# JeremyWesthead/deacon-server

Measured on AMD Instinct MI355X. Metric: Mbp/s filtered (k=31,w=15 vs panhuman-1-sized index), decisions bit-exact vs CPU, higher is better.
Workload: dtype u64

## Files before the change

deacon-server_amd/csrc/ctx.hip:

```cpp
#include "dcn_ctx.h"
#include "dcn_host_pool.h"

#include <atomic>
#include <cstdlib>
#include <cstring>
#include <mutex>
#include <new>

using dcn_host::HostPool;

uint32_t dcn_cu_count() {
    int dev = 0, cus = 256;
    if (hipGetDevice(&dev) == hipSuccess) (void)hipDeviceGetAttribute(&cus, hipDeviceAttributeMultiprocessorCount, dev);
    return (uint32_t)std::max(cus, 1);
}

namespace dcn_impl {

int alloc_records(dcn_ctx *c, uint64_t n_records) {
    n_records = (n_records + 63) / 64 * 64;
    if (n_records > (1ull << 29)) return dcn_fail(DCN_ERR_CAPACITY, "more than 2^29 hit records in global sets per batch: use smaller batches");
    if (c->d_set_slots) hipFree(c->d_set_slots);
    c->d_set_slots = nullptr;
    c->rec_capacity = 0;
    DCN_TRY(dev_alloc(&c->d_set_slots, 4 * n_records + 64, "set_slots"));
    c->rec_capacity = n_records;
    return DCN_OK;
}

void free_slot_buffers(dcn_slot &sl) {
    if (sl.owns_buffers) {
        void *dev[] = {sl.d_ascii, sl.d_packed, sl.d_invmask, sl.d_offsets, sl.d_unit_id, sl.d_keep, sl.d_hits, sl.d_total};
        for (void *p : dev)
            if (p) hipFree(p);
    }
    if (sl.d_report) hipFree(sl.d_report);
    if (sl.d_off32) hipFree(sl.d_off32);
    if (sl.d_mask_pairs) hipFree(sl.d_mask_pairs);
    void *host[] = {sl.h_keep, sl.h_hits, sl.h_total, sl.h_report, sl.h_off32, sl.h_mask_pairs};
    for (void *p : host)
        if (p) hipHostFree(p);
    if (sl.done) hipEventDestroy(sl.done);
    for (hipEvent_t e : sl.ev_h2d) hipEventDestroy(e);
    for (hipEvent_t e : sl.ev_comp) hipEventDestroy(e);
    sl = dcn_slot();
}

static void free_ctx(dcn_ctx *c) {
    if (!c) return;
    hipSetDevice(c->device);
    if (c->stream) hipStreamSynchronize(c->stream);
    if (c->copy_stream) hipStreamSynchronize(c->copy_stream);
    if (c->d2h_stream) hipStreamSynchronize(c->d2h_stream);
    if (c->pack_stream) {
        hipStreamSynchronize(c->pack_stream);
        hipStreamDestroy(c->pack_stream);
    }
    for (int i = 0; i < 2; ++i) {
        if (c->pack_done[i]) hipEventDestroy(c->pack_done[i]);
        if (c->buf_free[i]) hipEventDestroy(c->buf_free[i]);
    }
    if (c->plan_done) hipEventDestroy(c->plan_done);
    if (c->d_packed_b) hipFree(c->d_packed_b);
    if (c->d_invmask_b) hipFree(c->d_invmask_b);
    if (c->d_pack_status) hipFree(c->d_pack_status);
    for (auto &sl : c->slots) free_slot_buffers(sl);
    void *dev[] = {c->d_ascii, c->d_offsets, c->d_unit_id, c->d_packed, c->d_invmask,
                   c->d_read_tiles, c->d_read_tile_first, c->d_unit_first_read, c->d_unit_tile_first, c->d_unit_tile_count, c->d_tiles,
                   c->d_keep, c->d_unit_state, c->d_hits, c->d_total, c->d_unit_scratch, c->d_caps,
                   c->d_set_off, c->d_tile_hits, c->d_pending, c->d_big, c->d_rec_hash, c->d_set_slots, c->d_status, c->d_wave_kept, c->d_report, c->d_dump_hash,
                   c->d_dump_pos, c->d_dump_count, c->d_dump_valid, c->d_tile_read_pos,
                   c->d_cls_big, c->d_cls_n_big, c->d_cls_match, c->d_cls_hits, c->d_cls_total,
                   c->d_loc_bits, c->d_loc_labels, c->d_loc_counts, c->d_loc_big, c->d_loc_n_big, c->d_loc_block_sums,
                   c->d_loc_seg_offsets, c->d_loc_segs, c->d_trk_bin_offsets, c->d_trk_piece_offsets, c->d_trk_bins,
                   c->d_plc_words, c->d_plc_abits, c->d_plc_big, c->d_plc_n_big, c->d_plc_out,
                   c->d_pls_rbits, c->d_pls_n_rounds, c->d_pls_read_counts, c->d_pls_counts, c->d_pls_block_sums,
                   c->d_pls_offsets, c->d_pls_rounds, c->d_pls_out, c->d_ppr_out, c->d_ppr_hist, c->d_vfy_items, c->d_vfy_out,
                   c->d_aln_work, c->d_aln_n_ops, c->d_aln_trace, c->d_aln_slots, c->d_aln_cigar, c->d_aln_offsets, c->d_aln_block_sums};
    for (void *p : dev)
        if (p && !((char *)p >= c->d_slab && (char *)p < c->d_slab + c->slab_bytes)) hipFree(p);
    if (c->d_slab) hipFree(c->d_slab);
    for (int i = 0; i < dcn_ctx::N_STAGE; ++i) {
        if (c->h_stage[i]) hipHostFree(c->h_stage[i]);
        if (c->stage_free[i]) hipEventDestroy(c->stage_free[i]);
    }
    for (int i = 0; i < dcn_ctx::N_EV; ++i) {
        if (c->ev_h2d[i]) hipEventDestroy(c->ev_h2d[i]);
        if (c->ev_comp[i]) hipEventDestroy(c->ev_comp[i]);
    }
    if (c->h_report) hipHostFree(c->h_report);
    for (int i = 0; i < dcn_ctx::PROF_RING; ++i)
        for (int j = 0; j <= DCN_N_STAGES; ++j)
            if (c->prof_ev[i][j]) hipEventDestroy(c->prof_ev[i][j]);
    if (c->copy_done) hipEventDestroy(c->copy_done);
    if (c->stream) hipStreamDestroy(c->stream);
    if (c->copy_stream) hipStreamDestroy(c->copy_stream);
    if (c->d2h_stream) hipStreamDestroy(c->d2h_stream);
    delete c;
}

static int prof_harvest(dcn_ctx *c, int only_slot = -1) {
    for (int i = 0; i < dcn_ctx::PROF_RING; ++i) {
        if (!c->prof_used[i] || (only_slot >= 0 && i != only_slot)) continue;
        const int first = c->prof_scan_only[i] ? DCN_STAGE_SCAN : 0, last = c->prof_scan_only[i] ? DCN_STAGE_SCAN : DCN_N_STAGES - 1;
        DCN_HIP(hipEventSynchronize(c->prof_ev[i][last + 1]));
        for (int j = first; j <= last; ++j) {
            float ms = 0.f;
            DCN_HIP(hipEventElapsedTime(&ms, c->prof_ev[i][j], c->prof_ev[i][j + 1]));
            c->prof_ms[j] += ms;
        }
// ... 4 lines not shown
}

int prof_begin(dcn_ctx *c, int *slot) {
    *slot = -1;
    if (!c->profiling) return DCN_OK;
    int i = c->prof_next;
    c->prof_next = (i + 1) % dcn_ctx::PROF_RING;
    if (c->prof_used[i]) DCN_TRY(prof_harvest(c, i));
    for (int j = 0; j <= DCN_N_STAGES; ++j)
        if (!c->prof_ev[i][j]) DCN_HIP(hipEventCreate(&c->prof_ev[i][j]));
    c->prof_scan_only[i] = c->profiling == 2;
    if (c->profiling == 1) DCN_HIP(hipEventRecord(c->prof_ev[i][0], c->stream));
    *slot = i;
    return DCN_OK;
}

int check_params(const dcn_params *p) {
    if (!p) return dcn_fail(DCN_ERR_ARG, "params is NULL");
    if (p->reserved != 0) return dcn_fail(DCN_ERR_ARG, "params.reserved must be 0");
    if (p->deplete > 1) return dcn_fail(DCN_ERR_ARG, "params.deplete must be 0 or 1");
    return DCN_OK;
}

static bool ensure_pack_ahead(dcn_ctx *c) {
    if (c->pack_ahead_state != 0) return c->pack_ahead_state > 0;
    c->pack_ahead_state = -1;
    if (!getenv("DCN_PACK_AHEAD") || getenv("DCN_NO_PACK_AHEAD")) return false;
    int prio_low = 0, prio_high = 0;
    (void)hipDeviceGetStreamPriorityRange(&prio_low, &prio_high);
    bool ok = hipStreamCreateWithPriority(&c->pack_stream, hipStreamNonBlocking, prio_high) == hipSuccess;
    ok = ok && hipEventCreateWithFlags(&c->plan_done, hipEventDisableTiming) == hipSuccess;
    for (int i = 0; ok && i < 2; ++i)
        ok = hipEventCreateWithFlags(&c->pack_done[i], hipEventDisableTiming) == hipSuccess &&
             hipEventCreateWithFlags(&c->buf_free[i], hipEventDisableTiming) == hipSuccess;
    ok = ok && hipMalloc((void **)&c->d_packed_b, packed_words(c->max_bases) * sizeof(uint32_t)) == hipSuccess &&
         hipMalloc((void **)&c->d_invmask_b, mask_words(c->max_bases) * sizeof(uint32_t)) == hipSuccess &&
         hipMalloc((void **)&c->d_pack_status, 2 * sizeof(dcn_status)) == hipSuccess;
    if (ok) {
        ok = hipMemset(c->d_packed_b, 0, packed_words(c->max_bases) * sizeof(uint32_t)) == hipSuccess &&
             hipMemset(c->d_invmask_b, 0, mask_words(c->max_bases) * sizeof(uint32_t)) == hipSuccess &&
             hipDeviceSynchronize() == hipSuccess;
    }
    if (!ok) {
        (void)hipGetLastError();
        if (c->d_packed_b) hipFree(c->d_packed_b);
        if (c->d_invmask_b) hipFree(c->d_invmask_b);
        if (c->d_pack_status) hipFree(c->d_pack_status);
        c->d_packed_b = c->d_invmask_b = nullptr;
        c->d_pack_status = nullptr;
        return false;
    }
    c->pack_ahead_state = 1;
    return true;
}

static dcn_scan_args scan_args(const dcn_ctx *c, const dcn_index *index, uint32_t *packed, uint32_t *invmask, uint64_t stream_bases);

int enqueue_batch(dcn_ctx *c, const BatchView &v, const dcn_params *params, bool pack_ahead) {
    hipStream_t st = c->stream;
    const dcn_index *idx = c->index;
    if (c->scratch_dirty) DCN_HIP(hipMemsetAsync(c->d_unit_scratch, 0, (uint64_t)c->max_reads * 4 * sizeof(uint32_t), st));
    c->scratch_dirty = true;
    DCN_HIP(hipMemsetAsync(c->d_status, 0, sizeof(dcn_status), st));

    int prof_slot = -1;
    DCN_TRY(prof_begin(c, &prof_slot));
    uint32_t *packed = v.d_packed + DCN_FRONT_PAD, *invmask = v.d_invmask + DCN_FRONT_PAD;
    int ahead_buf = -1;
    const uint32_t *newline_flag = nullptr;
    bool short_fused = false;
    static const bool no_early_out = getenv("DCN_NO_EARLY_OUT") != nullptr, no_early_out_pairs = getenv("DCN_NO_EARLY_OUT_PAIRS") != nullptr;
    const bool decisions_only_call = !v.d_hits && !v.d_total && params->abs_threshold >= 1 && params->abs_threshold <= 4 && !no_early_out;
    if (v.d_ascii && pack_ahead && c->profiling != 1 && ensure_pack_ahead(c)) {
        ahead_buf = c->pack_buf;
        c->pack_buf ^= 1;
        if (ahead_buf == 1) {
            packed = c->d_packed_b + DCN_FRONT_PAD;
            invmask = c->d_invmask_b + DCN_FRONT_PAD;
        }
        dcn_status *ps = c->d_pack_status + ahead_buf;
        DCN_HIP(hipStreamWaitEvent(c->pack_stream, c->buf_free[ahead_buf], 0));
        if (!getenv("DCN_PACK_AHEAD_EARLY")) DCN_HIP(hipStreamWaitEvent(c->pack_stream, c->plan_done, 0));
        DCN_HIP(hipMemsetAsync(ps, 0, sizeof(dcn_status), c->pack_stream));
        DCN_TRY(dcn_launch_pack_beside(v.d_ascii, v.b0, v.b1, packed, invmask, ps, c->pack_stream));
        DCN_HIP(hipEventRecord(c->pack_done[ahead_buf], c->pack_stream));
        DCN_HIP(hipStreamWaitEvent(st, c->pack_done[ahead_buf], 0));
        newline_flag = &ps->any_newline;
    } else if (v.d_ascii) {
        short_fused = c->short_fused && !v.d_unit_id && params->prefix_length == 0 && v.b0 == 0 && v.b1 == v.stream_bases &&
                      v.n_reads == v.n_units && c->tile_windows >= dcn_short_lmax() && idx->variant == DCN_VARIANT_DEFAULT &&
                      dcn_scan_has_short_path(idx->k, idx->w) && !decisions_only_call;
        if (short_fused) DCN_TRY(dcn_launch_shape(v.d_offsets, v.n_reads, v.stream_bases, dcn_short_lmax(), c->d_status, st));
        DCN_TRY(dcn_launch_pack(v.d_ascii, v.b0, v.b1, packed, invmask, c->d_status, st));
    }
    DCN_PROF_MARK(DCN_STAGE_PACK);

    const uint32_t n_reads = v.n_reads, n_units = v.n_units;
    dcn_plan_args pa = plan_args(c, idx, v.d_ascii, v.d_offsets, v.d_unit_id, n_reads, n_units, params->prefix_length);
    pa.unit_base = v.unit_base;
    pa.unit_state = c->d_unit_state;
    pa.unit_scratch = c->d_unit_scratch;
    pa.scratch_stride = c->max_reads;
    pa.newline_flag = newline_flag;
    pa.stream_bases = v.stream_bases;
    pa.check_offsets = 1;
    pa.max_tiles = c->max_tiles;
    pa.short_armed = short_fused ? 1u : 0u;
    DCN_TRY(dcn_launch_plan(pa, st));
    if (pack_ahead && c->pack_ahead_state == 1) DCN_HIP(hipEventRecord(c->plan_done, st));
    DCN_PROF_MARK(DCN_STAGE_PLAN);

    const UnitScratch us = unit_scratch(c);
    dcn_scan_args sa = scan_args(c, idx, packed, invmask, v.stream_bases);
    sa.unit_tile_first = c->d_unit_tile_first;
    sa.unit_tile_count = c->d_unit_tile_count;
    sa.abs_threshold = params->abs_threshold;
    sa.rel_threshold = params->rel_threshold;
    sa.deplete = params->deplete;
    sa.early_out_max_items = 0;
    if (decisions_only_call) {
        uint32_t lo = 0, hi = 65535;
        while (lo < hi) {
            uint32_t mid = (lo + hi + 1) / 2;
            if (dcn_required_hits(params->abs_threshold, params->rel_threshold, mid) == params->abs_threshold) lo = mid;
            else hi = mid - 1;
        }
        sa.early_out_max_items = lo;
        sa.early_out_pairs = no_early_out_pairs ? 0u : 1u;
    }
    sa.keep = v.d_keep;
    sa.hits = v.d_hits;
    sa.total = v.d_total;
    sa.unit_state = c->d_unit_state;
    sa.g_total = us.g_total;
    sa.g_hitcnt = us.g_hitcnt;
    sa.g_zero = us.g_zero;
    sa.rec_hash = c->d_rec_hash;
    sa.rec_shift = c->rec_shift;
    sa.tile_windows = c->tile_windows;
    sa.tile_hits = c->d_tile_hits;
    sa.pending = c->d_pending;
    sa.status = c->d_status;
    sa.ascii = short_fused ? v.d_ascii : nullptr;
    sa.offsets = v.d_offsets;
    sa.n_reads = n_reads;
    sa.wave_kept = c->d_wave_kept;
    DCN_TRY(dcn_launch_scan(sa, tile_bound(c, n_reads, v.b1 - v.b0), false, st));
    DCN_PROF_MARK(DCN_STAGE_SCAN);

    const bool decisions_only = !v.d_hits && !v.d_total && !getenv("DCN_NO_EARLY_OUT");
    const dcn_distinct_args da = distinct_args(c, n_units, params, c->d_rec_hash, c->rec_shift, decisions_only ? us.g_total : nullptr);
    DCN_TRY(dcn_launch_distinct(da, st));
    DCN_PROF_MARK(DCN_STAGE_DISTINCT);

    dcn_finish_args fa = finish_args(c, n_units, params, v.d_unit_id ? c->d_unit_first_read : nullptr, v.d_offsets, v.d_keep,
                                     v.d_hits, v.d_total, v.d_report);
    fa.short_counted = short_fused ? 1u : 0u;
    fa.pending = c->d_pending;
    fa.wave_kept = c->d_wave_kept;
    DCN_TRY(dcn_launch_finish(fa, st));
    c->scratch_dirty = false;
    if (pack_ahead && c->pack_ahead_state == 1) DCN_HIP(hipEventRecord(c->buf_free[ahead_buf >= 0 ? ahead_buf : 0], st));
    DCN_PROF_MARK(DCN_STAGE_FINISH);
    if (prof_slot >= 0) c->prof_used[prof_slot] = true;
    return DCN_OK;
}

int grow_run_slots(dcn_ctx *c) {
    if (c->rec_shift == 0) return DCN_OK;
    const bool in_slab = c->d_rec_hash && (char *)c->d_rec_hash >= c->d_slab && (char *)c->d_rec_hash < c->d_slab + c->slab_bytes;
    if (c->d_rec_hash && !in_slab) hipFree(c->d_rec_hash);
    c->d_rec_hash = nullptr;
    const uint32_t old_shift = c->rec_shift;
    c->rec_shift = 0;
    int rc = dev_alloc(&c->d_rec_hash, c->max_bases + 128, "rec_hash (one slot per window)");
    if (rc != DCN_OK) {
        c->rec_shift = old_shift;
        int rc2 = dev_alloc(&c->d_rec_hash, (c->max_bases >> old_shift) + 256, "rec_hash");
        return rc2 != DCN_OK ? rc2 : rc;
    }
    static std::atomic<bool> said{false};
    if (!said.exchange(true) && getenv("DCN_QUIET") == nullptr)
        std::fprintf(stderr, "deacon-hip: a unit's hits outgrew its run of the record array; this context now keeps one slot per window "
                             "(%.2f GB instead of %.2f GB of device memory)\n", (c->max_bases + 128) * 8e-9,
                     ((c->max_bases >> old_shift) + 256) * 8e-9);
    return DCN_OK;
}

int overflow_error(const dcn_ctx *c, uint64_t need) {
    return dcn_fail(DCN_ERR_CAPACITY, "hit-record scratch overflow: need " + std::to_string(need) +
                                          " records, have " + std::to_string(c->rec_capacity) +
                                          " (dcn_ctx_reserve_records)");
}

int sync_and_check(dcn_ctx *c, uint64_t *needed_records) {
    DCN_HIP(hipStreamSynchronize(c->stream));
    if (needed_records) *needed_records = 0;
    if (c->profiling) DCN_TRY(prof_harvest(c));
    if (!c->batch_pending) return DCN_OK;
    c->batch_pending = false;
// ... 320 lines not shown
}

}

using namespace dcn_impl;

extern "C" int dcn_ctx_create(const dcn_index *index, uint64_t max_batch_bases, uint32_t max_batch_reads,
                              dcn_ctx **out) {
    if (!out) return dcn_fail(DCN_ERR_ARG, "out is NULL");
    *out = nullptr;
    if (!index) return dcn_fail(DCN_ERR_ARG, "index is NULL");
    if (max_batch_bases == 0 || max_batch_reads == 0) return dcn_fail(DCN_ERR_ARG, "batch limits must be > 0");
    if (max_batch_reads > 0xFFFFFF00u) return dcn_fail(DCN_ERR_ARG, "max_batch_reads too large");
    dcn_ctx *c = new (std::nothrow) dcn_ctx();
    if (!c) return dcn_fail(DCN_ERR_NOMEM, "host allocation failed");
    c->index = index;
    c->device = index->device;
    c->max_bases = max_batch_bases;
    c->max_reads = max_batch_reads;
    if (const char *tw = getenv("DCN_TILE_WINDOWS")) {
        long v = strtol(tw, nullptr, 10);
        if (v >= 16 && v <= (long)DCN_MAX_TILE_WINDOWS) c->tile_windows = (uint32_t)v;
    }
    uint64_t mt = (uint64_t)max_batch_reads + max_batch_bases / c->tile_windows + 1;
    if (mt > 0xFFFFFF00ull) {
        delete c;
        return dcn_fail(DCN_ERR_ARG, "batch limits imply more than 2^32 tiles");
    }
    c->max_tiles = (uint32_t)mt;
    c->chunk_bases = 64ull << 20;
    if (const char *cb = getenv("DCN_CHUNK_BASES")) {
        long long v = atoll(cb);
        if (v >= 1024) c->chunk_bases = (uint64_t)v;
    }
    int rc = DCN_OK;
    auto fail = [&](int code) {
        free_ctx(c);
        return code;
    };
    if (hipSetDevice(c->device) != hipSuccess) return fail(dcn_fail(DCN_ERR_HIP, "hipSetDevice failed"));
    bool ok = hipStreamCreateWithFlags(&c->stream, hipStreamNonBlocking) == hipSuccess &&
              hipStreamCreateWithFlags(&c->copy_stream, hipStreamNonBlocking) == hipSuccess &&
              hipStreamCreateWithFlags(&c->d2h_stream, hipStreamNonBlocking) == hipSuccess &&
              hipEventCreateWithFlags(&c->copy_done, hipEventDisableTiming) == hipSuccess;
    for (int i = 0; ok && i < dcn_ctx::N_STAGE; ++i)
        ok = hipEventCreateWithFlags(&c->stage_free[i], hipEventDisableTiming) == hipSuccess;
    for (int i = 0; ok && i < dcn_ctx::N_EV; ++i)
        ok = hipEventCreateWithFlags(&c->ev_h2d[i], hipEventDisableTiming) == hipSuccess &&
             hipEventCreateWithFlags(&c->ev_comp[i], hipEventDisableTiming) == hipSuccess;
    if (!ok) return fail(dcn_fail(DCN_ERR_HIP, "stream/event creation failed"));
    c->rec_shift = 2;
    if (index->w <= 7) c->rec_shift = 0;
    c->short_fused = getenv("DCN_NO_SHORT_FUSED") == nullptr;
    if (const char *rs = getenv("DCN_REC_SHIFT")) c->rec_shift = (uint32_t)std::min(3, std::max(0, atoi(rs)));
    uint64_t MR = max_batch_reads;
    const bool slab = getenv("DCN_CTX_SLAB") != nullptr;
    uint64_t slab_off = 0;
    for (int pass = slab ? 0 : 1; pass < 2; ++pass) {
        if (slab && pass == 1) {
            c->slab_bytes = slab_off;
            if (hipMalloc((void **)&c->d_slab, c->slab_bytes) != hipSuccess) {
                c->d_slab = nullptr;
                c->slab_bytes = 0;
                return fail(dcn_fail(DCN_ERR_NOMEM, "hipMalloc of the context slab failed"));
            }
            slab_off = 0;
        }
#define A(ptr, count, what)                                                                                   \
    if (slab) {                                                                                               \
        if (pass == 1) c->ptr = reinterpret_cast<decltype(c->ptr)>(c->d_slab + slab_off);                     \
        slab_off += (std::max<uint64_t>((count), 1) * sizeof(*c->ptr) + (2u << 20) - 1) / (2u << 20) * (2u << 20); \
    } else if ((rc = dev_alloc(&c->ptr, (count), what)) != DCN_OK)                                            \
        return fail(rc)
    A(d_ascii, max_batch_bases + 64, "ascii");
    A(d_offsets, MR + 1, "offsets");
    A(d_unit_id, MR, "unit_id");
    A(d_packed, packed_words(max_batch_bases), "packed");
    A(d_invmask, mask_words(max_batch_bases), "invmask");
    A(d_read_tiles, MR, "read_tiles");
    A(d_read_tile_first, MR + 1, "read_tile_first");
    A(d_unit_first_read, MR + 1, "unit_first_read");
    A(d_unit_tile_first, MR + 1, "unit_tile_first");
    A(d_unit_tile_count, MR + 1, "unit_tile_count");
    A(d_tiles, mt, "tiles");
    A(d_keep, MR, "keep");
    A(d_unit_state, MR, "unit_state");
    A(d_hits, MR, "hits");
    A(d_total, MR, "total");
    A(d_unit_scratch, MR * 4, "unit_scratch");
    A(d_caps, MR, "caps");
    A(d_set_off, MR + 1, "set_off");
    A(d_tile_hits, mt, "tile_hits");
    A(d_pending, MR, "pending");
    A(d_big, MR + mt / 64 + 1, "big");
    A(d_rec_hash, (max_batch_bases >> c->rec_shift) + 256, "rec_hash");
    A(d_status, 1, "status");
    A(d_wave_kept, MR / DCN_WAVE + 1, "wave_kept");
    A(d_report, 1, "report");
#undef A
    }
    uint64_t recs = std::min<uint64_t>(std::max<uint64_t>(max_batch_bases / 16, 1u << 16), 1ull << 29);
    if (const char *rc_env = getenv("DCN_RECORD_CAPACITY")) recs = std::min<uint64_t>(std::max<uint64_t>(strtoull(rc_env, nullptr, 10), 64), 1ull << 29);
    if ((rc = alloc_records(c, recs)) != DCN_OK) return fail(rc);
    c->stage_bytes = std::min<uint64_t>(std::max<uint64_t>(max_batch_bases + 64, 4096), 32ull << 20);
    if (const char *sb = getenv("DCN_STAGE_BYTES"))
        c->stage_bytes = std::min<uint64_t>(std::max<uint64_t>(strtoull(sb, nullptr, 10), 4096), 32ull << 20);
// ... 128 lines not shown
```

deacon-server_amd/csrc/dcn_ctx.h:

```cpp
#pragma once

#include "dcn_dump_sweep.h"
#include "dcn_internal.h"
#include "dcn_plan.h"

#include <algorithm>
#include <functional>
#include <vector>

struct dcn_split_round;
struct dcn_verify_item;
struct dcn_align_work;

struct dcn_mask_range {
    uint64_t g0 = 0, g1 = 0, pairs_off = 0;
    uint32_t n = 0;
};

struct dcn_chunk {
    uint32_t r0 = 0, r1 = 0, u0 = 0, u1 = 0;
    uint64_t b0 = 0, b1 = 0;
    uint64_t max_len = 0;
    std::vector<dcn_mask_range> mask_ranges;
};

struct dcn_slot {
    bool allocated = false, busy = false, owns_buffers = false;
    uint64_t ticket = 0;
    uint8_t *d_ascii = nullptr;
    uint32_t *d_packed = nullptr, *d_invmask = nullptr;
    uint64_t *d_offsets = nullptr;
    uint32_t *d_off32 = nullptr, *h_off32 = nullptr;
    bool off32 = false;
    bool lean = false;
    uint2 *d_mask_pairs = nullptr, *h_mask_pairs = nullptr;
    uint64_t mask_pairs_cap = 0, mask_pairs_used = 0;
    uint32_t *d_unit_id = nullptr;
    uint8_t *d_keep = nullptr;
    uint32_t *d_hits = nullptr, *d_total = nullptr;
    dcn_batch_report *d_report = nullptr;
    uint8_t *h_keep = nullptr;
    uint32_t *h_hits = nullptr, *h_total = nullptr;
    dcn_batch_report *h_report = nullptr;
    hipEvent_t done = nullptr;
    std::vector<hipEvent_t> ev_h2d, ev_comp;
    dcn_params params = {};
    bool device_pack = false;
    bool has_units = false, counts = false;
    uint32_t n_reads = 0, n_units = 0;
    uint64_t n_bases = 0;
    uint8_t *u_keep = nullptr;
    uint32_t *u_hits = nullptr, *u_total = nullptr;
    bool keep_direct = false, hits_direct = false, total_direct = false;
    std::vector<dcn_chunk> chunks;
};

struct dcn_ctx {
    const dcn_index *index = nullptr;
    int device = 0;
    hipStream_t stream = nullptr, copy_stream = nullptr, d2h_stream = nullptr;
    hipStream_t pack_stream = nullptr;
    uint32_t *d_packed_b = nullptr, *d_invmask_b = nullptr;
    dcn_status *d_pack_status = nullptr;
    hipEvent_t pack_done[2] = {}, buf_free[2] = {}, plan_done = nullptr;
    int pack_buf = 0, pack_ahead_state = 0;
    static constexpr int N_STAGE = 3, N_EV = 8, N_SLOTS = 2;
    hipEvent_t copy_done = nullptr, stage_free[N_STAGE] = {};
    hipEvent_t ev_h2d[N_EV] = {}, ev_comp[N_EV] = {};
    int ev_next = 0, stage_next = 0;
    uint64_t max_bases = 0;
    uint32_t max_reads = 0;
    uint32_t tile_windows = 256;
    uint32_t max_tiles = 0;
    uint64_t chunk_bases = 0;
    uint8_t *d_ascii = nullptr;
    uint64_t *d_offsets = nullptr;
    uint32_t *d_unit_id = nullptr;
    uint32_t *d_packed = nullptr, *d_invmask = nullptr;
    uint32_t *d_read_tiles = nullptr, *d_read_tile_first = nullptr;
    uint32_t *d_unit_first_read = nullptr, *d_unit_tile_first = nullptr, *d_unit_tile_count = nullptr;
    dcn_tile *d_tiles = nullptr;
    uint8_t *d_keep = nullptr, *d_unit_state = nullptr;
    uint32_t *d_hits = nullptr, *d_total = nullptr;
    uint32_t *d_unit_scratch = nullptr;
    bool scratch_dirty = false;
    uint32_t *d_caps = nullptr, *d_set_off = nullptr;
    uint64_t *d_rec_hash = nullptr;
    uint32_t rec_shift = 0;
    char *d_slab = nullptr;
    uint64_t slab_bytes = 0;
    uint32_t *d_tile_hits = nullptr, *d_pending = nullptr;
    uint2 *d_big = nullptr;
    uint64_t rec_capacity = 0;
    uint64_t *d_set_slots = nullptr;
    dcn_status *d_status = nullptr;
    unsigned long long *d_wave_kept = nullptr;
    bool short_fused = true;
    bool last_batch_short = false;
    dcn_batch_report *d_report = nullptr;
    dcn_batch_report *h_report = nullptr;
    uint64_t host_stats[DCN_N_STATS] = {};
    uint8_t *h_stage[N_STAGE] = {};
    uint64_t stage_bytes = 0;
    dcn_slot slots[N_SLOTS];
    uint64_t next_ticket = 1;
    uint64_t *d_dump_hash = nullptr;
    uint32_t *d_dump_pos = nullptr, *d_dump_count = nullptr, *d_tile_read_pos = nullptr;
    uint8_t *d_dump_valid = nullptr;
    uint32_t *d_cls_big = nullptr, *d_cls_n_big = nullptr;
    uint32_t *d_cls_match = nullptr, *d_cls_hits = nullptr, *d_cls_total = nullptr;
    uint32_t cls_hits_members = 0;
    uint32_t *d_loc_bits = nullptr, *d_loc_labels = nullptr;
    uint32_t *d_loc_counts = nullptr, *d_loc_big = nullptr, *d_loc_n_big = nullptr;
    unsigned long long *d_loc_block_sums = nullptr;
    uint64_t *d_loc_seg_offsets = nullptr;
    dcn_segment *d_loc_segs = nullptr;
    uint64_t loc_seg_cap = 0;
    uint64_t *d_trk_bin_offsets = nullptr, *d_trk_piece_offsets = nullptr;
// ... 183 lines not shown
```

deacon-server_amd/csrc/dcn_internal.h:

```cpp
#pragma once

#include <hip/hip_runtime.h>
#include <stdint.h>

#include <string>

#include "../../include/deacon_hip.h"

void dcn_set_error(const std::string &msg);
int dcn_fail(int code, const std::string &msg);

#define DCN_HIP(expr)                                                                              \
    do {                                                                                           \
        hipError_t _e = (expr);                                                                    \
        if (_e != hipSuccess)                                                                      \
            return dcn_fail(_e == hipErrorOutOfMemory ? DCN_ERR_NOMEM : DCN_ERR_HIP,               \
                            std::string(#expr) + ": " + hipGetErrorString(_e));                    \
    } while (0)

inline int dcn_hip_fail(hipError_t e, const char *what) {
    return dcn_fail(e == hipErrorOutOfMemory ? DCN_ERR_NOMEM : DCN_ERR_HIP, std::string(what) + ": " + hipGetErrorString(e));
}

template <typename F>
// ... 112 lines not shown
    uint32_t short_batch;
    unsigned long long need;
    unsigned long long stats[DCN_N_STATS];
};

struct dcn_scan_args {
    const uint32_t *packed;
    const uint32_t *invmask;
    dcn_tile *tiles;
    const uint32_t *tile_read_pos;
    const uint32_t *n_tiles;
    uint32_t *unit_tile_first;
    uint32_t *unit_tile_count;
    dcn_table_view table;
    uint32_t k, w;
    uint64_t stream_bases;
    uint64_t abs_threshold;
    double rel_threshold;
    uint32_t deplete;
    uint32_t early_out_max_items;
    uint32_t early_out_pairs;
    uint8_t *keep;
    uint32_t *hits, *total;
    uint8_t *unit_state;
    uint32_t *g_total;
    uint32_t *g_hitcnt;
    uint32_t *g_zero;
    uint64_t *rec_hash;
    uint32_t rec_shift;
    uint32_t tile_windows;
    uint32_t *tile_hits;
    uint32_t *pending;
    dcn_status *status;
    uint64_t *dump_hash;
    uint32_t *dump_pos;
    uint8_t *dump_valid;
    uint32_t *dump_count;
    uint32_t dump_abs;
    uint32_t variant;
    uint32_t nt_rot;
    uint32_t cmp_mask;
    uint32_t nt_combine_xor;
    const uint8_t *ascii;
    const uint64_t *offsets;
    uint32_t n_reads;
    unsigned long long *wave_kept;
};

int dcn_launch_pack(const uint8_t *d_ascii, uint64_t base_begin, uint64_t base_end, uint32_t *d_packed,
                    uint32_t *d_invmask, dcn_status *status, hipStream_t stream, bool index_side = false,
                    uint32_t block_threads = 256);
int dcn_launch_pack_beside(const uint8_t *d_ascii, uint64_t base_begin, uint64_t base_end, uint32_t *d_packed, uint32_t *d_invmask,
                           dcn_status *status, hipStream_t stream);
int dcn_launch_scan(const dcn_scan_args &args, uint32_t max_tiles, bool dump, hipStream_t stream);
bool dcn_scan_has_short_path(uint32_t k, uint32_t w);
uint32_t dcn_short_lmax();
int dcn_launch_shape(const uint64_t *d_offsets, uint32_t n_reads, uint64_t stream_bases, uint32_t lmax, dcn_status *status,
                     hipStream_t stream);

int dcn_table_build(dcn_index *idx, const uint64_t *host_keys, uint64_t n);
int dcn_table_contains(const dcn_index *idx, const uint64_t *host_keys, uint64_t n, uint8_t *out);
int dcn_table_contains_device(const dcn_index *idx, const uint64_t *d_keys, uint64_t n, uint8_t *d_out,
                              hipStream_t stream);
int dcn_table_probe_ceiling(const dcn_index *idx, const uint64_t *d_keys, uint64_t n, uint32_t reps, double *best,
                            hipStream_t stream);
int dcn_table_insert_varint9(dcn_index *idx, const uint64_t *d_raw, uint64_t n, unsigned long long *d_new,
                             uint32_t *d_zero, uint32_t *d_bad, hipStream_t stream);
uint64_t dcn_table_groups_for(uint64_t n_keys);
int dcn_table_alloc(dcn_index *idx, uint64_t n_keys_capacity);
int dcn_table_reserve(dcn_index *idx, uint64_t n_keys_capacity);
int dcn_table_insert_dump(dcn_index *idx, const uint64_t *d_hash, const uint8_t *d_valid, const uint32_t *d_abs_pos,
                          uint64_t n_slots, const uint8_t *d_ascii, float entropy_threshold, hipStream_t stream);
int dcn_table_count_valid(const uint8_t *d_valid, uint64_t n, uint64_t *count, hipStream_t stream);
int dcn_table_export(const dcn_index *idx, uint64_t *host_out, uint64_t capacity, uint64_t *n_out);
int dcn_table_merge(dcn_index *dst, const dcn_index *src, const dcn_index *minus);
hipError_t dcn_table_malloc(uint64_t **p, uint64_t bytes);
int dcn_table_clone_by_keys(const dcn_index *src, dcn_index *dst);


__host__ __device__ inline uint64_t dcn_required_hits(uint64_t abs_threshold, double rel_threshold,
                                                      uint64_t total) {
    uint64_t rel_required = 0;
    if (total != 0) {
        double r = round(rel_threshold * (double)total);
        if (!(r > 0.0)) rel_required = 0;
        else if (r >= 18446744073709551616.0) rel_required = ~0ull;
        else rel_required = (uint64_t)r;
        if (rel_required < 1) rel_required = 1;
    }
    return abs_threshold > rel_required ? abs_threshold : rel_required;
}

__host__ __device__ inline bool dcn_decide(uint64_t hits, uint64_t total, uint64_t abs_threshold,
                                           double rel_threshold, uint32_t deplete) {
    uint64_t required = dcn_required_hits(abs_threshold, rel_threshold, total);
    return deplete ? (hits < required) : (hits >= required);
}
```

deacon-server_amd/csrc/plan.hip:

```cpp
#include "dcn_internal.h"
#include "dcn_plan.h"
#include "dcn_probe.h"
#include "dcn_short_lane.h"

#include <algorithm>

namespace {

__device__ inline uint32_t effective_windows(const uint8_t *ascii, uint64_t off, uint64_t len, uint64_t prefix,
                                             uint32_t k, uint32_t l) {
    if (len < k) return 0;
    const uint64_t n = (prefix > 0 && len > prefix) ? prefix : len;
    const bool nl = ascii && n > 0 && ascii[off + n - 1] == '\n';
    return dcn_window_count(len, n, nl, k, l);
}

__device__ inline void write_tile(const dcn_plan_args &a, uint32_t first, uint32_t j, uint64_t off, uint32_t nwin,
                                  uint32_t unit, bool whole_unit = false) {
    uint32_t wstart = j * a.tile_windows;
    uint32_t carry = j > 0 ? 1u : 0u;
    if (a.check_offsets && first + j >= a.max_tiles) {
        a.status->bad_offsets = 1;
        return;
    }
// ... 88 lines not shown
            a.read_tiles[r] = nt[c];
            a.read_tile_first[r] = first;
        }
        uint32_t u = r;
        bool unit_head = true;
        if (a.unit_id) {
            u = a.unit_id[r] - a.unit_base;
            if (a.check_offsets) {
                const uint32_t prev = r ? a.unit_id[r - 1] : a.unit_base - 1u;
                if (u >= a.n_units || a.unit_id[r] - prev > 1u || (r == a.n_reads - 1 && u != a.n_units - 1)) {
                    a.status->bad_offsets = 1;
                    if (u >= a.n_units) u = 0;
                }
            }
            unit_head = r == 0 || a.unit_id[r - 1] != a.unit_id[r];
            if (unit_head) a.unit_first_read[u] = r;
            if (r == a.n_reads - 1) a.unit_first_read[a.n_units] = a.n_reads;
        }
        if (unit_head) {
            uint32_t count = nt[c];
            if (a.unit_id) {
                uint32_t q = r + 1;
                while (q < a.n_reads && a.unit_id[q] - a.unit_base == u) {
                    if (q >= block_end) {
                        count = 0xFFFFFFFFu;
                        break;
                    }
                    count += s_tiles[q - block_first];
                    ++q;
                }
            }
            if (a.unit_id || nt[c] != 1) {
                a.unit_tile_first[u] = first;
                a.unit_tile_count[u] = count;
            }
            if (a.unit_state) a.unit_state[u] = 0;
        }
        const uint64_t off = a.offsets[r];
        for (uint32_t j = 0; j < min(nt[c], OWN); ++j) write_tile(a, first, j, off, nwin[c], u, !a.unit_id && nt[c] == 1);
        if (nt[c] > OWN) long_reads[atomicAdd(&n_long, 1u)] = c * 256 + tid;
    }
    __syncthreads();
    for (uint32_t q = 0; q < n_long; ++q) {
        const uint32_t li = long_reads[q], lr = block_first + li;
        const uint32_t lnt = s_tiles[li], lfirst = s_first[li];
        uint32_t lu = a.unit_id ? a.unit_id[lr] - a.unit_base : lr;
        if (a.check_offsets && lu >= a.n_units) lu = 0;
        const uint64_t loff = a.offsets[lr];
        const uint32_t lnwin = effective_windows(ascii, loff, a.offsets[lr + 1] - loff, a.prefix_length, a.k, a.k + a.w - 1);
        for (uint32_t j = OWN + tid; j < lnt; j += blockDim.x) write_tile(a, lfirst, j, loff, lnwin, lu);
    }
}

__global__ __launch_bounds__(256) void shape_kernel(const uint64_t *__restrict__ offsets, uint32_t n_reads, uint64_t stream_bases,
                                                    uint32_t lmax, dcn_status *status) {
    bool bad = false;
    const uint32_t stride = gridDim.x * blockDim.x;
    for (uint32_t r0 = blockIdx.x * blockDim.x + threadIdx.x; r0 < n_reads; r0 += 4 * stride) {
        uint64_t off[4], end[4];
#pragma unroll
        for (int q = 0; q < 4; ++q) {
            const uint32_t r = r0 + q * stride;
            off[q] = end[q] = 0;
            if (r < n_reads && r >= r0) {
                off[q] = offsets[r];
                end[q] = offsets[r + 1];
            }
        }
#pragma unroll
        for (int q = 0; q < 4; ++q) bad |= end[q] < off[q] || end[q] > stream_bases || end[q] - off[q] > lmax;
    }
    const int any_bad = __syncthreads_or(bad ? 1 : 0);
    if (threadIdx.x == 0) {
        if (any_bad) atomicOr(&status->shape_bad, 1u);
        __threadfence();
        const bool last = atomicAdd(&status->shape_done, 1u) == gridDim.x - 1;
        if (last && atomicOr(&status->shape_bad, 0u) == 0u) status->short_batch = 1;
    }
}

#ifndef DCN_LDS_SET_LOG2
#define DCN_LDS_SET_LOG2 11
#endif
constexpr uint32_t DCN_LDS_SET_SLOTS = 1u << DCN_LDS_SET_LOG2;
constexpr uint32_t DCN_LDS_SET_MAX = DCN_LDS_SET_SLOTS * 7 / 10 - 33;
constexpr uint32_t DCN_LDS_WALK_MAX_TILES = 1024;

__device__ inline uint32_t set_slot_of(uint64_t h, uint32_t cap) {
    uint32_t lo = (uint32_t)h, hi = (uint32_t)(h >> 32);
    return ((lo ^ ((hi << 13) | (hi >> 19))) * 0x85EBCA6Bu) & (cap - 1);
}

__global__ __launch_bounds__(64) void unit_distinct_kernel(dcn_distinct_args a) {
    __shared__ unsigned long long set[DCN_LDS_SET_SLOTS];
    if (a.status->run_overflow) return;
    const uint32_t NP = a.status->n_pending;
    const uint32_t lane = threadIdx.x;
    uint32_t nu = 0, nfirst = 0, ncount = 0, nH = 0, ntot = 0;
    auto fetch = [&](uint32_t i) {
        if (i < NP) {
            nu = a.pending[i];
            nfirst = a.unit_tile_first[nu];
            ncount = a.unit_tile_count[nu];
            nH = a.g_hitcnt[nu];
            ntot = a.g_total ? a.g_total[nu] : 0u;
        }
    };
    fetch(blockIdx.x);
    for (uint32_t i = blockIdx.x; i < NP; i += gridDim.x) {
        const uint32_t u = nu, first = nfirst, count = ncount, H = nH, tot = ntot;
        fetch(i + gridDim.x);
        if (H == 0) {
            if (lane == 0) a.caps[u] = 0;
            continue;
        }
        uint32_t enough = 0xFFFFFFFFu;
        if (a.g_total) {
            const uint64_t req = dcn_required_hits(a.abs_threshold, a.rel_threshold, tot);
            if ((uint64_t)H < req) {
                if (lane == 0) {
                    a.g_distinct[u] = 0;
                    a.caps[u] = 0;
                }
                continue;
// ... 347 lines not shown
                }
                a.g_zero[lo] = 1;
            }
        } else if (!dcn_table_contains_dev(a.table, h)) {
            a.hashes[i] = 0;
        }
    }
}

__global__ __launch_bounds__(256) void hash_units_kernel(dcn_probe_hashes_args a) {
    uint32_t u = blockIdx.x * blockDim.x + threadIdx.x;
    if (u == 0) {
        *a.n_tiles = a.n_units;
        a.status->any_records = 1;
        a.status->n_pending = a.n_units;
    }
    if (u >= a.n_units) return;
    const uint64_t n = a.hash_offsets[u + 1] - a.hash_offsets[u];
    dcn_tile t;
    t.scan_start = a.hash_offsets[u];
    t.unit = u;
    t.nwf = (uint32_t)n & 0x3FFFFFFFu;
    a.tiles[u] = t;
    a.tile_hits[u] = (uint32_t)n;
    a.unit_tile_first[u] = u;
    a.unit_tile_count[u] = 1;
    a.unit_state[u] = 0;
    a.pending[u] = u;
    a.g_total[u] = (uint32_t)n;
    a.g_hitcnt[u] = (uint32_t)n;
    a.g_distinct[u] = 0;
    a.g_zero[u] = 0;
}

inline uint32_t blocks_for(uint64_t n, uint32_t cap = 256 * 16) {
    uint64_t b = (n + 255) / 256;
    if (b < 1) b = 1;
    return (uint32_t)(b > cap ? cap : b);
}

}

int dcn_launch_plan(const dcn_plan_args &a, hipStream_t stream) {
    if (a.n_reads >= (1u << 19))
        hipLaunchKernelGGL(plan_kernel<8>, dim3((a.n_reads + 2047) / 2048), dim3(256), 0, stream, a);
    else
        hipLaunchKernelGGL(plan_kernel<1>, dim3((a.n_reads + 255) / 256), dim3(256), 0, stream, a);
    DCN_HIP(hipGetLastError());
    return DCN_OK;
}

int dcn_launch_shape(const uint64_t *d_offsets, uint32_t n_reads, uint64_t stream_bases, uint32_t lmax, dcn_status *status,
                     hipStream_t stream) {
    hipLaunchKernelGGL(shape_kernel, dim3(blocks_for((n_reads + 3) / 4, 2048)), dim3(256), 0, stream, d_offsets, n_reads, stream_bases,
                       lmax, status);
    DCN_HIP(hipGetLastError());
    return DCN_OK;
}

int dcn_launch_distinct(const dcn_distinct_args &a, hipStream_t stream) {
    hipLaunchKernelGGL(unit_distinct_kernel, dim3(std::max(1u, std::min(a.n_units, 256u * 10u))), dim3(64), 0, stream, a);
    hipLaunchKernelGGL(distinct_clear_kernel, dim3(1024), dim3(256), 0, stream, a.set_slots, a.set_capacity, a.status);
    hipLaunchKernelGGL(big_insert_kernel, dim3(2048), dim3(256), 0, stream, a);
    DCN_HIP(hipGetLastError());
    return DCN_OK;
}

int dcn_launch_finish(const dcn_finish_args &a, hipStream_t stream) {
    hipLaunchKernelGGL(finish_kernel, dim3(blocks_for(a.n_units, 1024)), dim3(256), 0, stream, a);
    DCN_HIP(hipGetLastError());
    return DCN_OK;
}

int dcn_launch_probe_hashes(const dcn_probe_hashes_args &a, hipStream_t stream) {
    hipLaunchKernelGGL(hash_units_kernel, dim3((a.n_units + 255) / 256), dim3(256), 0, stream, a);
    if (a.n_hashes)
        hipLaunchKernelGGL(probe_hashes_kernel, dim3(blocks_for(a.n_hashes)), dim3(256), 0, stream, a);
    DCN_HIP(hipGetLastError());
    return DCN_OK;
}
```

deacon-server_amd/csrc/scan.hip:

```cpp
#include "dcn_internal.h"
#include "dcn_probe.h"

#include "dcn_pack.h"
#include "dcn_short_lane.h"

#include <atomic>
#include <type_traits>

namespace {

__device__ __constant__ uint32_t NT_F[4] = {0x95c60474u, 0x62a02b4cu, 0x82572324u, 0x4be24456u};

__device__ inline uint32_t rotl32(uint32_t x, uint32_t r) { return __funnelshift_l(x, x, r); }

#ifndef DCN_WAVE_OPS_SHFL
#define DCN_WAVE_OPS_SHFL 0
#endif
template <bool MAX>
__device__ inline uint32_t wave_scan_dpp(uint32_t v) {
    auto op = [](uint32_t x, uint32_t y) { return MAX ? max(x, y) : x + y; };
    v = op(v, (uint32_t)__builtin_amdgcn_update_dpp(0, (int)v, 0x111, 0xf, 0xf, false));
    v = op(v, (uint32_t)__builtin_amdgcn_update_dpp(0, (int)v, 0x112, 0xf, 0xf, false));
    v = op(v, (uint32_t)__builtin_amdgcn_update_dpp(0, (int)v, 0x114, 0xf, 0xf, false));
    v = op(v, (uint32_t)__builtin_amdgcn_update_dpp(0, (int)v, 0x118, 0xf, 0xf, false));
// ... 968 lines not shown
    const dcn_short_span sp = dcn_short_lane(off, end, nl, a.k, W, a16);
    const int64_t c0 = __shfl((long long)sp.chunk_first, 0, 64);
    const int64_t c1 = __shfl((long long)sp.chunk_last, (int)n_have - 1, 64);
    const uint32_t words = (uint32_t)min((int64_t)DCN_STAGE_WORDS, max((int64_t)0, c1 - c0 + 1));
    for (uint32_t i0 = 0; i0 < words; i0 += 4 * DCN_WAVE) {
        uint4 v[4];
#pragma unroll
        for (int q = 0; q < 4; ++q) {
            const uint32_t i = i0 + q * DCN_WAVE + lane;
            v[q] = make_uint4(0, 0, 0, 0);
            if (i < words) v[q] = load_chunk(c0 + i);
        }
#pragma unroll
        for (int q = 0; q < 4; ++q) {
            const uint32_t i = i0 + q * DCN_WAVE + lane;
            if (i < words) {
                sh.stage_p[i] = dcn_pack4(v[q].x) | (dcn_pack4(v[q].y) << 8) | (dcn_pack4(v[q].z) << 16) | (dcn_pack4(v[q].w) << 24);
                sh.stage_m16[i] = (uint16_t)(dcn_invalid4(v[q].x) | (dcn_invalid4(v[q].y) << 4) | (dcn_invalid4(v[q].z) << 8) |
                                             (dcn_invalid4(v[q].w) << 12));
            }
        }
    }
    sh.read_len[lane] = have ? (uint32_t)(end - off) : 0u;
    ShortLane sl;
    sl.have = have;
    sl.windows = have ? sp.windows : 0u;
    sl.s_local = have ? (uint32_t)((int64_t)(a16 + off) - 16 * c0) : 16u;
    __syncthreads();
    scan_body<W, false, false, false, false, true>(a, sh, sl);
}

#ifndef DCN_SHORT_FUSED
#define DCN_SHORT_FUSED 1
#endif
template <int W>
constexpr bool dcn_scan_has_short = DCN_SHORT_FUSED && DCN_LIST_BY_LANE && !DCN_EXPORT_UNIFORM && W == 15;

template <int W, bool K128, bool DUMP, bool FAST, bool VAR = false, bool SHORTK = false>
__global__ __launch_bounds__(DCN_WAVE, FAST ? DCN_MIN_WAVES_FAST : DCN_MIN_WAVES) void scan_kernel(dcn_scan_args a) {
    if constexpr (SHORTK) {
        static_assert(dcn_scan_has_short<W> && !K128 && !DUMP && !FAST && !VAR, "the short path is a counting kernel of fixed w, k <= 32");
        __shared__ WaveSharedShort sh;
        if (a.status->short_batch) scan_short<W>(a, sh);
    } else {
        __shared__ WaveShared sh;
        if constexpr (dcn_scan_has_short<W> && !K128 && !DUMP && !FAST && !VAR) {
            if (a.ascii && a.status->short_batch) return;
        }
        scan_body<W, K128, DUMP, FAST, VAR, false>(a, sh, ShortLane{});
    }
}

template <int W, bool VAR = false>
int launch_w(const dcn_scan_args &args, uint32_t blocks, bool dump, bool k128, size_t dyn, hipStream_t stream) {
#define DCN_LAUNCH(K128_, DUMP_, FAST_)                                                               \
    do {                                                                                              \
        auto kern = scan_kernel<W, K128_, DUMP_, FAST_ && !VAR, VAR>;                                 \
        if (dyn > 0) {                                                                                \
            hipError_t e = hipFuncSetAttribute(reinterpret_cast<const void *>(kern),                  \
                                               hipFuncAttributeMaxDynamicSharedMemorySize, (int)dyn); \
            if (e != hipSuccess) return dcn_fail(DCN_ERR_HIP, std::string("dyn LDS: ") + hipGetErrorString(e)); \
        }                                                                                             \
        hipLaunchKernelGGL(kern, dim3(blocks), dim3(DCN_WAVE), dyn, stream, args);                    \
    } while (0)
    const bool fast = !dump && args.early_out_max_items != 0;
    if constexpr (dcn_scan_has_short<W> && !VAR) {
        if (args.ascii && !k128 && !dump && !fast && args.n_reads)
            hipLaunchKernelGGL((scan_kernel<W, false, false, false, false, true>), dim3((args.n_reads + DCN_WAVE - 1) / DCN_WAVE),
                               dim3(DCN_WAVE), 0, stream, args);
    }
    if (k128) {
        if (dump) DCN_LAUNCH(true, true, false);
        else if (fast) DCN_LAUNCH(true, false, true);
        else DCN_LAUNCH(true, false, false);
    } else {
        if (dump) DCN_LAUNCH(false, true, false);
        else if (fast) DCN_LAUNCH(false, false, true);
        else DCN_LAUNCH(false, false, false);
    }
#undef DCN_LAUNCH
    DCN_HIP(hipGetLastError());
    return DCN_OK;
}

}

namespace {
std::atomic<uint32_t> g_variant{DCN_VARIANT_DEFAULT};
}

uint32_t dcn_current_variant() { return g_variant.load(); }

int dcn_set_minimizer_variant(uint32_t nt_rot, uint32_t cmp_bits, uint32_t combine) {
    if (nt_rot < 1 || nt_rot > 31) return dcn_fail(DCN_ERR_ARG, "minimizer variant: rotation must be 1..31");
    if (cmp_bits != 16 && cmp_bits != 32) return dcn_fail(DCN_ERR_ARG, "minimizer variant: 16 or 32 hash bits are compared");
    if (combine > 1) return dcn_fail(DCN_ERR_ARG, "minimizer variant: combine is 0 (fw + rc) or 1 (fw ^ rc)");
    g_variant.store((nt_rot << 16) | (cmp_bits << 8) | combine);
    return DCN_OK;
}

int dcn_get_minimizer_variant(uint32_t *nt_rot, uint32_t *cmp_bits, uint32_t *combine) {
    const uint32_t v = g_variant.load();
    if (nt_rot) *nt_rot = v >> 16;
    if (cmp_bits) *cmp_bits = (v >> 8) & 0xFF;
    if (combine) *combine = v & 0xFF;
    return DCN_OK;
}

bool dcn_scan_has_short_path(uint32_t k, uint32_t w) { return k <= 32 && w == 15 && dcn_scan_has_short<15>; }
uint32_t dcn_short_lmax() { return DCN_SHORT_LMAX; }

int dcn_launch_scan(const dcn_scan_args &args_in, uint32_t max_tiles, bool dump, hipStream_t stream) {
    if (max_tiles == 0) return DCN_OK;
    uint32_t blocks = (max_tiles + DCN_WAVE - 1) / DCN_WAVE;
    bool k128 = args_in.k > 32;
    const uint32_t v = args_in.variant ? args_in.variant : DCN_VARIANT_DEFAULT;
    if (v != DCN_VARIANT_DEFAULT) {
        dcn_scan_args args = args_in;
        args.nt_rot = v >> 16;
        args.cmp_mask = ((v >> 8) & 0xFF) == 32 ? 0xFFFFFFFFu : 0xFFFF0000u;
        args.nt_combine_xor = v & 0xFF;
        args.early_out_max_items = 0;
        if (args.w > 128) return dcn_fail(DCN_ERR_ARG, "minimizer variant: w <= 128 (two u64 keys per window slot in LDS)");
        size_t dyn = (size_t)args.w * DCN_WAVE * sizeof(ulonglong2);
        return launch_w<0, true>(args, blocks, dump, k128, dyn, stream);
    }
    const dcn_scan_args &args = args_in;
    switch (args.w) {
    case 15: return launch_w<15>(args, blocks, dump, k128, 0, stream);
    case 11: return launch_w<11>(args, blocks, dump, k128, 0, stream);
    case 1: return launch_w<1>(args, blocks, dump, k128, 0, stream);
    default: {
        size_t dyn = (size_t)args.w * DCN_WAVE * sizeof(uint2);
        return launch_w<0>(args, blocks, dump, k128, dyn, stream);
    }
    }
}
```

Before: 463,000.

## Fork short-read and classic scan kernels onto concurrent streams; vectorise shape check

The short-read scan kernel and the classic tiled scan kernel were launched back to back on one stream. They now run concurrently: the short kernel stays on the main stream and the classic kernel goes to a forked, by default low-priority, stream joined by events. This only happens when the short path is armed, profiling is off and enough blocks are involved. Separately, the offsets shape-validation kernel now reads 16-byte pairs per lane with wave shuffles and a capped grid, cutting load count and launch width. The fork adds event and stream overhead and possible contention between the two kernels.

```diff
diff --git a/deacon-server_amd/csrc/ctx.hip b/deacon-server_amd/csrc/ctx.hip
--- a/deacon-server_amd/csrc/ctx.hip
+++ b/deacon-server_amd/csrc/ctx.hip
@@ -1,5 +1,6 @@
 #include "dcn_ctx.h"
 #include "dcn_host_pool.h"
+#include "dcn_scan_fork.h"
 
 #include <atomic>
 #include <cstdlib>
@@ -56,6 +57,12 @@
         hipStreamSynchronize(c->pack_stream);
         hipStreamDestroy(c->pack_stream);
     }
+    if (c->fork_stream) {
+        hipStreamSynchronize(c->fork_stream);
+        hipStreamDestroy(c->fork_stream);
+    }
+    if (c->ev_fork) hipEventDestroy(c->ev_fork);
+    if (c->ev_classic) hipEventDestroy(c->ev_classic);
     for (int i = 0; i < 2; ++i) {
         if (c->pack_done[i]) hipEventDestroy(c->pack_done[i]);
         if (c->buf_free[i]) hipEventDestroy(c->buf_free[i]);
@@ -166,6 +173,42 @@
     }
     c->pack_ahead_state = 1;
     return true;
+}
+
+static bool ensure_scan_fork(dcn_ctx *c) {
+    if (c->scan_fork_state != 0) return c->scan_fork_state > 0;
+    c->scan_fork_state = -1;
+    if (!c->scan_fork) return false;
+    int prio_low = 0, prio_high = 0;
+    (void)hipDeviceGetStreamPriorityRange(&prio_low, &prio_high);
+    bool ok = hipStreamCreateWithPriority(&c->fork_stream, hipStreamNonBlocking, c->scan_fork_low_priority ? prio_low : 0) == hipSuccess;
+    ok = ok && hipEventCreateWithFlags(&c->ev_fork, hipEventDisableTiming) == hipSuccess &&
+         hipEventCreateWithFlags(&c->ev_classic, hipEventDisableTiming) == hipSuccess;
+    if (!ok) {
+        (void)hipGetLastError();
+        if (c->fork_stream) hipStreamDestroy(c->fork_stream);
+        if (c->ev_fork) hipEventDestroy(c->ev_fork);
+        if (c->ev_classic) hipEventDestroy(c->ev_classic);
+        c->fork_stream = nullptr;
+        c->ev_fork = c->ev_classic = nullptr;
+        return false;
+    }
+    c->scan_fork_state = 1;
+    return true;
+}
+
+static int launch_scan_forked(dcn_ctx *c, const dcn_scan_args &sa, uint32_t max_tiles) {
+    DCN_HIP(hipEventRecord(c->ev_fork, c->stream));
+    DCN_HIP(hipStreamWaitEvent(c->fork_stream, c->ev_fork, 0));
+    int rc = dcn_launch_scan(sa, max_tiles, false, c->stream, DCN_SCAN_SHORT_ONLY);
+    if (rc == DCN_OK) rc = dcn_launch_scan(sa, max_tiles, false, c->fork_stream, DCN_SCAN_CLASSIC_ONLY);
+    hipError_t e = hipEventRecord(c->ev_classic, c->fork_stream);
+    if (e == hipSuccess) e = hipStreamWaitEvent(c->stream, c->ev_classic, 0);
+    if (e != hipSuccess) {
+        (void)hipStreamSynchronize(c->fork_stream);
+        if (rc == DCN_OK) rc = dcn_hip_fail(e, "scan fork: join");
+    }
+    return rc;
 }
 
 static dcn_scan_args scan_args(const dcn_ctx *c, const dcn_index *index, uint32_t *packed, uint32_t *invmask, uint64_t stream_bases);
@@ -259,7 +302,13 @@
     sa.offsets = v.d_offsets;
     sa.n_reads = n_reads;
     sa.wave_kept = c->d_wave_kept;
-    DCN_TRY(dcn_launch_scan(sa, tile_bound(c, n_reads, v.b1 - v.b0), false, st));
+    const uint32_t scan_tiles = tile_bound(c, n_reads, v.b1 - v.b0);
+    const uint32_t idle_blocks = std::min(dcn_scan_blocks(scan_tiles), (n_reads + DCN_WAVE - 1) / DCN_WAVE);
+    if (dcn_scan_fork_wanted(short_fused, c->profiling, idle_blocks, c->scan_fork_min_blocks, c->scan_fork) &&
+        ensure_scan_fork(c))
+        DCN_TRY(launch_scan_forked(c, sa, scan_tiles));
+    else
+        DCN_TRY(dcn_launch_scan(sa, scan_tiles, false, st));
     DCN_PROF_MARK(DCN_STAGE_SCAN);
 
     const bool decisions_only = !v.d_hits && !v.d_total && !getenv("DCN_NO_EARLY_OUT");
@@ -686,6 +735,10 @@
     c->rec_shift = 2;
     if (index->w <= 7) c->rec_shift = 0;
     c->short_fused = getenv("DCN_NO_SHORT_FUSED") == nullptr;
+    c->scan_fork = getenv("DCN_NO_SCAN_FORK") == nullptr;
+    c->scan_fork_min_blocks = DCN_SCAN_FORK_MIN_BLOCKS_DEFAULT;
+    if (const char *mb = getenv("DCN_SCAN_FORK_MIN_BLOCKS")) c->scan_fork_min_blocks = (uint32_t)std::min<unsigned long long>(strtoull(mb, nullptr, 10), 0xFFFFFFFFull);
+    if (const char *pr = getenv("DCN_SCAN_FORK_PRIORITY")) c->scan_fork_low_priority = strcmp(pr, "normal") != 0;
     if (const char *rs = getenv("DCN_REC_SHIFT")) c->rec_shift = (uint32_t)std::min(3, std::max(0, atoi(rs)));
     uint64_t MR = max_batch_reads;
     const bool slab = getenv("DCN_CTX_SLAB") != nullptr;
diff --git a/deacon-server_amd/csrc/dcn_ctx.h b/deacon-server_amd/csrc/dcn_ctx.h
--- a/deacon-server_amd/csrc/dcn_ctx.h
+++ b/deacon-server_amd/csrc/dcn_ctx.h
@@ -64,6 +64,12 @@
     dcn_status *d_pack_status = nullptr;
     hipEvent_t pack_done[2] = {}, buf_free[2] = {}, plan_done = nullptr;
     int pack_buf = 0, pack_ahead_state = 0;
+    hipStream_t fork_stream = nullptr;
+    hipEvent_t ev_fork = nullptr, ev_classic = nullptr;
+    int scan_fork_state = 0;
+    bool scan_fork = true;
+    bool scan_fork_low_priority = true;
+    uint32_t scan_fork_min_blocks = 0;
     static constexpr int N_STAGE = 3, N_EV = 8, N_SLOTS = 2;
     hipEvent_t copy_done = nullptr, stage_free[N_STAGE] = {};
     hipEvent_t ev_h2d[N_EV] = {}, ev_comp[N_EV] = {};
diff --git a/deacon-server_amd/csrc/dcn_internal.h b/deacon-server_amd/csrc/dcn_internal.h
--- a/deacon-server_amd/csrc/dcn_internal.h
+++ b/deacon-server_amd/csrc/dcn_internal.h
@@ -188,7 +188,9 @@
                     uint32_t block_threads = 256);
 int dcn_launch_pack_beside(const uint8_t *d_ascii, uint64_t base_begin, uint64_t base_end, uint32_t *d_packed, uint32_t *d_invmask,
                            dcn_status *status, hipStream_t stream);
-int dcn_launch_scan(const dcn_scan_args &args, uint32_t max_tiles, bool dump, hipStream_t stream);
+enum dcn_scan_part { DCN_SCAN_BOTH, DCN_SCAN_SHORT_ONLY, DCN_SCAN_CLASSIC_ONLY };
+int dcn_launch_scan(const dcn_scan_args &args, uint32_t max_tiles, bool dump, hipStream_t stream, dcn_scan_part part = DCN_SCAN_BOTH);
+uint32_t dcn_scan_blocks(uint32_t max_tiles);
 bool dcn_scan_has_short_path(uint32_t k, uint32_t w);
 uint32_t dcn_short_lmax();
 int dcn_launch_shape(const uint64_t *d_offsets, uint32_t n_reads, uint64_t stream_bases, uint32_t lmax, dcn_status *status,
diff --git a/deacon-server_amd/csrc/dcn_scan_fork.h b/deacon-server_amd/csrc/dcn_scan_fork.h
--- /dev/null
+++ b/deacon-server_amd/csrc/dcn_scan_fork.h
@@ -0,0 +1,9 @@
+#pragma once
+
+#include <stdint.h>
+
+constexpr uint32_t DCN_SCAN_FORK_MIN_BLOCKS_DEFAULT = 65536;
+
+inline bool dcn_scan_fork_wanted(bool armed, int profiling, uint32_t idle_blocks, uint32_t min_blocks, bool enabled) {
+    return enabled && armed && profiling != 1 && idle_blocks >= min_blocks;
+}
diff --git a/deacon-server_amd/csrc/plan.hip b/deacon-server_amd/csrc/plan.hip
--- a/deacon-server_amd/csrc/plan.hip
+++ b/deacon-server_amd/csrc/plan.hip
@@ -164,24 +164,39 @@
     }
 }
 
+constexpr uint32_t SHAPE_PAIRS = 8, SHAPE_CHUNK = SHAPE_PAIRS * 128, SHAPE_MAX_BLOCKS = 512;
 __global__ __launch_bounds__(256) void shape_kernel(const uint64_t *__restrict__ offsets, uint32_t n_reads, uint64_t stream_bases,
                                                     uint32_t lmax, dcn_status *status) {
     bool bad = false;
-    const uint32_t stride = gridDim.x * blockDim.x;
-    for (uint32_t r0 = blockIdx.x * blockDim.x + threadIdx.x; r0 < n_reads; r0 += 4 * stride) {
-        uint64_t off[4], end[4];
-#pragma unroll
-        for (int q = 0; q < 4; ++q) {
-            const uint32_t r = r0 + q * stride;
-            off[q] = end[q] = 0;
-            if (r < n_reads && r >= r0) {
-                off[q] = offsets[r];
-                end[q] = offsets[r + 1];
-            }
-        }
-#pragma unroll
-        for (int q = 0; q < 4; ++q) bad |= end[q] < off[q] || end[q] > stream_bases || end[q] - off[q] > lmax;
-    }
+    auto check = [&](uint64_t off, uint64_t end) { bad |= end < off || end > stream_bases || end - off > lmax; };
+    const uint64_t n_words = (uint64_t)n_reads + 1;
+    const uint32_t lead = (uint32_t)(((uintptr_t)offsets >> 3) & 1u);
+    const uint64_t n_chunks = (n_words - lead + SHAPE_CHUNK - 1) / SHAPE_CHUNK;
+    const uint32_t lane = threadIdx.x & 63;
+    const uint64_t wave = (uint64_t)blockIdx.x * (blockDim.x >> 6) + (threadIdx.x >> 6), n_waves = (uint64_t)gridDim.x * (blockDim.x >> 6);
+    for (uint64_t c = wave; c < n_chunks; c += n_waves) {
+        const uint64_t first = lead + c * SHAPE_CHUNK;
+        if (first + SHAPE_CHUNK < n_words) {
+            const ulonglong2 *p = reinterpret_cast<const ulonglong2 *>(offsets + first) + lane;
+            ulonglong2 v[SHAPE_PAIRS];
+#pragma unroll
+            for (uint32_t q = 0; q < SHAPE_PAIRS; ++q) v[q] = p[q * 64];
+            unsigned long long behind = 0;
+            if (lane == 63) behind = offsets[first + SHAPE_CHUNK];
+#pragma unroll
+            for (uint32_t q = 0; q < SHAPE_PAIRS; ++q) {
+                unsigned long long next = __shfl_down(v[q].x, 1, 64);
+                const uint32_t qn = q + 1 < SHAPE_PAIRS ? q + 1 : q;
+                const unsigned long long head = __shfl(v[qn].x, 0, 64);
+                if (lane == 63) next = q + 1 < SHAPE_PAIRS ? head : behind;
+                check(v[q].x, v[q].y);
+                check(v[q].y, next);
+            }
+        } else {
+            for (uint64_t i = first + lane; i + 1 < n_words && i < first + SHAPE_CHUNK; i += 64) check(offsets[i], offsets[i + 1]);
+        }
+    }
+    if (lead && n_reads && wave == 0 && lane == 0) check(offsets[0], offsets[1]);
     const int any_bad = __syncthreads_or(bad ? 1 : 0);
     if (threadIdx.x == 0) {
         if (any_bad) atomicOr(&status->shape_bad, 1u);
@@ -635,8 +650,9 @@
 
 int dcn_launch_shape(const uint64_t *d_offsets, uint32_t n_reads, uint64_t stream_bases, uint32_t lmax, dcn_status *status,
                      hipStream_t stream) {
-    hipLaunchKernelGGL(shape_kernel, dim3(blocks_for((n_reads + 3) / 4, 2048)), dim3(256), 0, stream, d_offsets, n_reads, stream_bases,
-                       lmax, status);
+    const uint64_t n_chunks = ((uint64_t)n_reads + SHAPE_CHUNK) / SHAPE_CHUNK;
+    hipLaunchKernelGGL(shape_kernel, dim3((uint32_t)std::min<uint64_t>((n_chunks + 3) / 4, SHAPE_MAX_BLOCKS)), dim3(256), 0, stream, d_offsets,
+                       n_reads, stream_bases, lmax, status);
     DCN_HIP(hipGetLastError());
     return DCN_OK;
 }
diff --git a/deacon-server_amd/csrc/scan.hip b/deacon-server_amd/csrc/scan.hip
--- a/deacon-server_amd/csrc/scan.hip
+++ b/deacon-server_amd/csrc/scan.hip
@@ -1044,7 +1044,7 @@
 }
 
 template <int W, bool VAR = false>
-int launch_w(const dcn_scan_args &args, uint32_t blocks, bool dump, bool k128, size_t dyn, hipStream_t stream) {
+int launch_w(const dcn_scan_args &args, uint32_t blocks, bool dump, bool k128, size_t dyn, hipStream_t stream, dcn_scan_part part) {
 #define DCN_LAUNCH(K128_, DUMP_, FAST_)                                                               \
     do {                                                                                              \
         auto kern = scan_kernel<W, K128_, DUMP_, FAST_ && !VAR, VAR>;                                 \
@@ -1057,11 +1057,12 @@
     } while (0)
     const bool fast = !dump && args.early_out_max_items != 0;
     if constexpr (dcn_scan_has_short<W> && !VAR) {
-        if (args.ascii && !k128 && !dump && !fast && args.n_reads)
+        if (part != DCN_SCAN_CLASSIC_ONLY && args.ascii && !k128 && !dump && !fast && args.n_reads)
             hipLaunchKernelGGL((scan_kernel<W, false, false, false, false, true>), dim3((args.n_reads + DCN_WAVE - 1) / DCN_WAVE),
                                dim3(DCN_WAVE), 0, stream, args);
     }
-    if (k128) {
+    if (part == DCN_SCAN_SHORT_ONLY) {
+    } else if (k128) {
         if (dump) DCN_LAUNCH(true, true, false);
         else if (fast) DCN_LAUNCH(true, false, true);
         else DCN_LAUNCH(true, false, false);
@@ -1101,10 +1102,11 @@
 
 bool dcn_scan_has_short_path(uint32_t k, uint32_t w) { return k <= 32 && w == 15 && dcn_scan_has_short<15>; }
 uint32_t dcn_short_lmax() { return DCN_SHORT_LMAX; }
-
-int dcn_launch_scan(const dcn_scan_args &args_in, uint32_t max_tiles, bool dump, hipStream_t stream) {
+uint32_t dcn_scan_blocks(uint32_t max_tiles) { return (max_tiles + DCN_WAVE - 1) / DCN_WAVE; }
+
+int dcn_launch_scan(const dcn_scan_args &args_in, uint32_t max_tiles, bool dump, hipStream_t stream, dcn_scan_part part) {
     if (max_tiles == 0) return DCN_OK;
-    uint32_t blocks = (max_tiles + DCN_WAVE - 1) / DCN_WAVE;
+    uint32_t blocks = dcn_scan_blocks(max_tiles);
     bool k128 = args_in.k > 32;
     const uint32_t v = args_in.variant ? args_in.variant : DCN_VARIANT_DEFAULT;
     if (v != DCN_VARIANT_DEFAULT) {
@@ -1115,16 +1117,16 @@
         args.early_out_max_items = 0;
         if (args.w > 128) return dcn_fail(DCN_ERR_ARG, "minimizer variant: w <= 128 (two u64 keys per window slot in LDS)");
         size_t dyn = (size_t)args.w * DCN_WAVE * sizeof(ulonglong2);
-        return launch_w<0, true>(args, blocks, dump, k128, dyn, stream);
+        return launch_w<0, true>(args, blocks, dump, k128, dyn, stream, part);
     }
     const dcn_scan_args &args = args_in;
     switch (args.w) {
-    case 15: return launch_w<15>(args, blocks, dump, k128, 0, stream);
-    case 11: return launch_w<11>(args, blocks, dump, k128, 0, stream);
-    case 1: return launch_w<1>(args, blocks, dump, k128, 0, stream);
+    case 15: return launch_w<15>(args, blocks, dump, k128, 0, stream, part);
+    case 11: return launch_w<11>(args, blocks, dump, k128, 0, stream, part);
+    case 1: return launch_w<1>(args, blocks, dump, k128, 0, stream, part);
     default: {
         size_t dyn = (size_t)args.w * DCN_WAVE * sizeof(uint2);
-        return launch_w<0>(args, blocks, dump, k128, dyn, stream);
-    }
-    }
-}
+        return launch_w<0>(args, blocks, dump, k128, dyn, stream, part);
+    }
+    }
+}
```

Result: faster. 471,100, median of 6 (+1.8%).
